# hormes/koordinator

Measured on AMD Instinct MI355X. Metric: pod×node Filter+Score evals/sec + pods/sec at 50k nodes, 1/2/4/8 GPUs, higher is better.
Workload: dtype int64

## Files before the change

koordinator_amd/csrc/gs_commit_spec.hip:

```cpp
#include <hip/hip_runtime.h>
#include <stdint.h>

#include "gs_eval_dev.h"

namespace gs {

constexpr int SP_WAVES = 8, SP_THREADS = 64 * SP_WAVES;
constexpr int SP_LAG = 12;
constexpr int SP_RES0 = 2, SP_NRES = 2;
constexpr int SP_RS0 = SP_RES0 + SP_NRES, SP_TABLES = SP_WAVES - SP_RS0;
constexpr int SP_W_VERIFY = 4;
__device__ __forceinline__ int sp_reserve_index(int wv) { return wv == 2 ? 0 : wv == 3 ? 1 : -1; }
__device__ __forceinline__ int sp_rescore_index(int wv) { return wv == 1 ? 0 : wv >= 5 ? wv - 4 : -1; }
constexpr int SP_JOBQ = 24;
constexpr int SP_HASH = 128;
static_assert(SP_HASH >= MAX_BATCH && (SP_HASH & (SP_HASH - 1)) == 0,
              "the node -> slot hash must hold every dirty slot (its insertion probes until a free entry)");
constexpr int SP_FRESH = 1, SP_FITERR = 2, SP_SLOW = 4, SP_OFFSHARD = 8;
constexpr int SP_PRED_GE = 16, SP_PRED_GT = 32;
constexpr uint32_t SP_SPIN_LIMIT = 1u << 24;
constexpr int SP_NST = 62, SP_STRIDE = 64;
constexpr int16_t SO_UNKNOWN = -2;
constexpr int16_t SO_UNLISTED = -3;

// ... 146 lines not shown
  int32_t* hkey = L.hkey;
  int16_t* hval = L.hval;
  Job* jobq = L.jobq;

  const uint64_t rt0 = __builtin_amdgcn_s_memrealtime();
  if (a.prev && a.prev[1] != 1) {
    if (tid == 0) { a.committed[0] = -1; a.committed[1] = 0; a.committed[3] = 0; a.committed[4] = 0; }
    return;
  }
  if (a.xerr && a.xerr[0]) {
    if (tid == 0) { a.committed[0] = 0; a.committed[1] = 0; a.committed[2] = 0; a.committed[3] = COMMIT_ERR_XTAG; a.committed[4] = 0; }
    return;
  }
  for (int i = tid; i < B; i += SP_THREADS) {
    pods(i) = a.pods[i];
    done_ver[i] = -1;
    has_row[i] = 0;
    rescored[i] = 0;
    jobs_left[i] = 0;
    jobs_all[i] = 0;
    resv[i] = 0;
  }
  for (int i = tid; i < SP_HASH; i += SP_THREADS) { hkey[i] = -1; hval[i] = -1; }
  for (int i = tid; i < B; i += SP_THREADS) tiebreak_records(a.seed, a.seq[i], a.tb + (size_t)i * TB_N);
  if (tid == 0) {
    s_decided = 0; s_stop = 0; s_parked = 0; s_finish = 0; s_cut_at = -1; s_err = 0; s_werr = 0;
    for (int k = 0; k < SP_NRES; ++k) { s_jq_head[k] = 0; s_jq_tail[k] = 0; }
    s_verified = 0; s_rb_req = 0; s_end_at = B; s_vend = -1; s_vcut = 0;
    s_committed = 0; s_hostcut = 0; s_nd = 0;
    s_snap = 0; s_prep_done = 0; s_reprep = 0;
  }
  __syncthreads();


  auto load_hdr = [&](int p, Hdr& o) {
    const LevelHdr* h = hdr_ptr(a, 0, p);
    const LevelExt* x = reinterpret_cast<const LevelExt*>(a.xbase + (size_t)a.bmax * LCAP * 4 +
                                                          (size_t)a.bmax * sizeof(LevelHdr)) + p;
    o.nlev = x->nlev;
    o.feas = h->feasible;
    o.next = x->next;
    o.hs = lane < MAXLEV ? h->score[lane] : lane < LEVALL ? x->score[lane - MAXLEV] : -1;
    o.hc = lane < MAXLEV ? h->count[lane] : lane < LEVALL ? x->count[lane - MAXLEV] : 0;
    o.lh = list_ptr(a, 0, p)[lane];
    o.tbv = a.tb[(size_t)p * TB_N + (lane & (TB_N - 1))];
  };
  auto tb_pos = [&](int p, int32_t tbv, int64_t T) -> int64_t {
// ... 1362 lines not shown
      for (int i = lane; i < (int)(sizeof(CpuStateDev) / 8); i += 64) d2[i] = s2[i];
      WAVE_FENCE();
    }
  }
  __syncthreads();
  const int nd = s_err ? 0 : s_nd, committed = s_err ? 0 : s_committed;
  for (int e = tid; e < nd * ROW_I64; e += SP_THREADS) {
    const int s = e / ROW_I64, j = e % ROW_I64;
    if (has_row[s] && row_word_mutable(j)) m.c64(kRowCol[j])[drows[s].node] = reinterpret_cast<const int64_t*>(&drows[s])[j];
  }
  for (int s = tid; s < nd; s += SP_THREADS)
    if (has_row[s]) m.c32(C_FREE_PODS)[drows[s].node] = drows[s].free_pods;
  constexpr int NW = 8 + 11 + 11 + 1;
  if (numa_on)
    for (int e = tid; e < nd * NW; e += SP_THREADS) {
      const int sl = e / NW, j = e % NW;
      if (!has_row[sl]) continue;
      const uint32_t node = drows[sl].node;
      if (j < 8) m.c64(C_ZRAW_CPU0 + j)[node] = (&drows[sl].nr.zraw_cpu[0])[j];
      else if (j < 19) m.c32(C_NFLAGS2 + (j - 8))[node] = reinterpret_cast<const int32_t*>(&drows[sl].nr.nflags2)[j - 8];
      else if (j < 30) m.c64(C_CPU_UN0 + (j - 19))[node] = reinterpret_cast<const int64_t*>(&cst[sl])[j - 19];
      else m.c32(C_CPU_META)[node] = (int32_t)cst[sl].meta;
    }
  for (int i = tid; i < committed; i += SP_THREADS) a.out[i].feasible = (uint32_t)final_F[i];
  if (ST && lane == 0)
    for (int i = 0; i < SP_NST; ++i)
      if (st_acc[i])
        atomicAdd(reinterpret_cast<unsigned long long*>(&a.stamps[wv * SP_STRIDE + i]), (unsigned long long)st_acc[i]);
  if (tid == 0) {
    a.committed[0] = committed;
    a.committed[1] = (committed == B && !s_hostcut && !s_err) ? 1 : 0;
    a.committed[2] = s_endwhy;
    a.committed[3] = s_err;
    a.committed[4] = (int32_t)(__builtin_amdgcn_s_memrealtime() - rt0);
  }
}

template <bool STAMPS, bool SPLIT>
static void spec_launch(const CommitArgs& a, hipStream_t st) {
  hipLaunchKernelGGL((commit_spec_kernel<STAMPS, SPLIT>), dim3(1), dim3(SP_THREADS), spec_smem_bytes(a.npods), st, a);
}

hipError_t launch_commit_spec(const CommitArgs& a, hipStream_t st) {
  const bool split = a.nranks <= 1 && a.npods >= 32;
  if (a.stamps) {
    if (split) spec_launch<true, true>(a, st);
// ... 26 lines not shown
```

koordinator_amd/csrc/gs_engine.cpp:

```cpp
#include <hip/hip_runtime.h>
#include <rccl/rccl.h>

#include <algorithm>
#include <chrono>
#include <cmath>
#include <cstdarg>
#include <cstdio>
#include <cstdlib>
#include <cstring>
#include <map>
#include <string>
#include <unordered_map>
#include <unordered_set>
#include <vector>
#include <condition_variable>
#include <deque>
#include <memory>
#include <mutex>
#include <thread>
#include <atomic>

#include "../../include/gpuscore.h"
#include "gs_ext.h"
#include "gs_kernels.h"
// ... 130 lines not shown
  PlacementDev* h_out = nullptr;
  int32_t* h_committed = nullptr;
  uint32_t* h_stage_idx = nullptr;
  int64_t* h_stage_rows = nullptr;
  uint8_t* h_xchg_send = nullptr;
  uint8_t* h_xchg_recv = nullptr;
  hipEvent_t ev[8] = {};
  struct Slot {
    int16_t* d_S = nullptr;
    uint8_t* d_aff = nullptr;
    hipEvent_t ev_go = nullptr, ev_evdone = nullptr;
    PodVec* d_pods = nullptr;
    uint64_t* d_seq = nullptr;
    PlacementDev* d_out = nullptr;
    int32_t* d_committed = nullptr;
    PodVec* h_pods = nullptr;
    uint64_t* h_seq = nullptr;
    PlacementDev* h_out = nullptr;
    int32_t* h_committed = nullptr;
    hipEvent_t ev[6] = {};
    bool untimed = false;
    uint8_t* d_lst = nullptr;
    uint32_t* d_hist = nullptr;
  } slot[2];
  bool cand_overlap = false;
  uint8_t* d_lst = nullptr;
  uint32_t* d_hist = nullptr;
  uint32_t* d_cscratch = nullptr;
  int cur_slot = 0;
  std::vector<HostNode> nodes;
  std::vector<uint8_t> row_dirty;
  std::vector<uint32_t> dirty_list;
  std::unordered_map<uint64_t, uint32_t> uid_node;
  std::unordered_map<uint64_t, int> metric_names;
  int64_t now = 0;
  bool prep_stale = true;
  Profile pf{};
  int max_score = 0;
  int nranks = 1, rank = 0;
  uint32_t n0 = 0, n1 = 0;
  bool sgather = false;
  uint32_t e0 = 0, e1 = 0;
  uint32_t sx_per = 0, sx_pld = 0;
  size_t sx_bytes = 0;
  uint8_t* d_sx_send = nullptr;
  uint8_t* d_sx_recv = nullptr;
// ... 927 lines not shown
    if (c->cb) {
      HIP_TRY(c, hipHostMalloc(&c->h_sx_send, c->sx_bytes, hipHostMallocDefault));
      HIP_TRY(c, hipHostMalloc(&c->h_sx_recv, c->sx_bytes * c->nranks, hipHostMallocDefault));
    }
  }
  if (!c->d_xsmall) HIP_TRY(c, hipMalloc(&c->d_xsmall, XSMALL * (1 + MAX_RANKS)));
  if (!c->h_xsmall) HIP_TRY(c, hipHostMalloc(&c->h_xsmall, XSMALL * MAX_RANKS, hipHostMallocDefault));
  if (const char* sk = env_str("GS_DEBUG_XCHG_SKEW")) {
    long r = -1;
    unsigned long long b = 0;
    if (sscanf(sk, "%ld:%llu", &r, &b) == 2) { c->dbg_xskew_rank = r; c->dbg_xskew_batch = b; }
  }
  return GS_OK;
}


void bind_slot(gs_ctx* c, int s) {
  const gs_ctx::Slot& x = c->slot[s];
  c->d_S = x.d_S; c->d_aff = x.d_aff;
  c->d_pods = x.d_pods; c->d_seq = x.d_seq; c->d_out = x.d_out; c->d_committed = x.d_committed;
  c->h_pods = x.h_pods; c->h_seq = x.h_seq; c->h_out = x.h_out; c->h_committed = x.h_committed;
  for (int i = 0; i < 6; ++i) c->ev[i] = x.ev[i];
  c->d_lst = x.d_lst; c->d_hist = x.d_hist;
  c->cur_slot = s;
}

constexpr int GS_REDO = 1;
constexpr size_t COMMITTED_BYTES = 32;

constexpr int SHORT_BATCH = 32;
bool direct_batch(const gs_ctx* c, int b, bool speculative) {
  return !speculative && b <= SHORT_BATCH && lvl_ranks(c) == 1;
}

bool cand_overlapped(const gs_ctx* c) {
  return c->cand_overlap && lvl_ranks(c) == 1 && !c->window_k && c->d_lst;
}

CommitArgs commit_args(gs_ctx* c, int b) {
  CommitArgs a{};
  a.m = c->mv;
  a.pods = c->d_pods;
  a.seq = c->d_seq;
  a.npods = b;
  a.nranks = lvl_ranks(c);
  a.shard_size = (c->N + a.nranks - 1) / a.nranks;
  a.xbase = a.nranks == 1 ? (cand_overlapped(c) ? c->d_lst : c->d_xchg_send)
                            : commit_spec_selected(c->window_k) ? c->d_xmerged : c->d_xchg_recv;
  a.xblock = c->xchg_bytes;
  a.bmax = c->B;
  a.pf = c->pf;
  a.seed = c->cfg.seed;
  a.forced_node = -1;
  a.out = c->d_out;
  a.committed = c->d_committed;
  a.stamps = c->d_stamps;
  a.topos = c->d_topos;
  a.aff = c->d_aff;
  a.ld = c->ld;
  a.own0 = c->n0;
  a.own1 = c->n1;
  a.S = a.nranks == 1 ? c->d_S : nullptr;
  a.S_own = c->d_S;
  a.window_k = c->window_k;
  a.start = c->next_start;
  a.nnodes = c->N;
  a.tb = c->d_tb;
  a.xerr = c->sgather ? c->d_xerr + (XERR_BYTES / 4) * c->cur_slot : c->nranks > 1 ? c->d_xerr : nullptr;
  return a;
}

int launch_batch(gs_ctx* c, int b, const int32_t* prev, const PlacementDev* prev_out = nullptr, int prev_b = 0) {
  const bool ovl = cand_overlapped(c);
  uint8_t* lblk = ovl ? c->d_lst : c->d_xchg_send;
  uint32_t* d_lists = reinterpret_cast<uint32_t*>(lblk);
  LevelHdr* d_hdrs = reinterpret_cast<LevelHdr*>(lblk + lists_bytes(c->B, c->lstride));
  LevelExt* d_ext = reinterpret_cast<LevelExt*>(lblk + lists_bytes(c->B, c->lstride) + (size_t)c->B * sizeof(LevelHdr));
  int prod_cols = 0;
  for (int i = 0; i < b; ++i) prod_cols |= (c->h_pods[i].flags & PF_PROD_SCORE) ? 1 : 0;
  uint32_t len = c->n1 - c->n0;
  if (c->numa_on && (c->numa_idx_stale || c->numa_idx_lo != c->e0 || c->numa_idx_hi != c->e1)) {
    std::vector<uint32_t> idx;
    for (uint32_t n = c->e0; n < c->e1; ++n)
      if (c->numa[n].cfg.numa_topology_policy != GS_NUMA_POLICY_NONE) idx.push_back(n);
    if (c->d_numa_idx) {
      HIP_TRY(c, host_wait_stream(c->st));
      HIP_TRY(c, host_wait_stream(c->st_ev));
      (void)hipFree(c->d_numa_idx);
      c->d_numa_idx = nullptr;
    }
// ... 21 lines not shown
  hipStream_t se = direct ? c->st : c->st_ev;
  hipStream_t rb = b >= SHORT_BATCH ? c->st_rb : c->st;
  const bool untimed = direct && rb == c->st;
  c->slot[c->cur_slot].untimed = untimed;
  if (!untimed) HIP_TRY(c, hipEventRecord(c->ev[0], se));
  if (c->sgather) {
    const uint32_t pld = c->sx_pld;
    uint8_t* blk = c->d_sx_send + c->sx_bytes * c->cur_slot;
    uint8_t* rcv = c->d_sx_recv + c->sx_bytes * c->nranks * c->cur_slot;
    HIP_TRY(c, launch_eval(c->mv, c->d_pods, b, c->pf, c->e0, c->e1, reinterpret_cast<int16_t*>(blk), pld, prod_cols,
                           c->d_numa_idx, c->numa_n, blk + (size_t)b * pld * 2, se, c->st2, c->ev_fork, c->ev_join,
                           c->slab_mv.i64 ? &c->slab_mv : nullptr));
    if (!untimed) HIP_TRY(c, hipEventRecord(c->ev[1], se));
    const size_t bytes = ((size_t)b * pld * 3 + sizeof(XTag) + 255) / 256 * 256;
    if (int rc = exchange(c, XSITE_SCORES, blk, rcv, bytes, nullptr, se)) return rc;
    HIP_TRY(c, launch_unpack_scores(rcv, bytes, c->nranks, b, c->sx_per, pld, c->N, c->d_S, c->d_aff, c->ld,
                                    c->d_xerr + (XERR_BYTES / 4) * c->cur_slot, se));
  } else {
    HIP_TRY(c, launch_eval(c->mv, c->d_pods, b, c->pf, c->n0, c->n1, c->d_S, c->ld, prod_cols, c->d_numa_idx, c->numa_n,
                           c->d_aff, se, c->st2, c->ev_fork, c->ev_join, c->slab_mv.i64 ? &c->slab_mv : nullptr));
    if (!untimed) HIP_TRY(c, hipEventRecord(c->ev[1], se));
  }
  const bool fix = ovl && prev && prev_b > 0;
  if (ovl) {
    CandPatch cp{};
    cp.extra = fix ? prev_b : 0;
    cp.hist = fix ? c->d_hist : nullptr;
    HIP_TRY(c, launch_cand(c->d_S, c->ld, len, c->n0, b, c->max_score, c->lstride, d_lists, d_hdrs, d_ext, se, &cp,
                           c->d_cscratch));
  }
  if (!direct) {
    HIP_TRY(c, hipEventRecord(sl.ev_evdone, c->st_ev));
    HIP_TRY(c, hipStreamWaitEvent(c->st, sl.ev_evdone, 0));
  } else {
    HIP_TRY(c, hipEventRecord(sl.ev_evdone, c->st));
    HIP_TRY(c, hipStreamWaitEvent(c->st_ev, sl.ev_evdone, 0));
  }
  if (fix) {
    CandPatch cp{c->mv, c->d_pods, c->pf, c->n0, c->n1, prod_cols, 0, c->d_aff, prev_out, prev};
    cp.extra = prev_b;
    cp.hist = c->d_hist;
    HIP_TRY(c, launch_fix_levels(c->d_S, c->ld, b, c->max_score, c->lstride, d_lists, d_hdrs, d_ext, cp, c->st));
  }
  const bool fused = prev && prev_b > 0 && !c->window_k;
  if (!ovl && prev && !fused)
    HIP_TRY(c, launch_patch(c->mv, c->d_pods, b, c->pf, c->n0, c->n1, c->d_S, c->ld, prod_cols, c->d_aff, prev_out,
                            prev, prev_b, c->st));
  if (!c->window_k && !ovl) {
    CandPatch cp{c->mv, c->d_pods, c->pf, c->n0, c->n1, prod_cols, 1, c->d_aff, prev_out, prev};
    HIP_TRY(c, launch_cand(c->d_S, c->ld, len, c->n0, b, c->max_score, c->lstride, d_lists, d_hdrs, d_ext, c->st,
                           fused ? &cp : nullptr, c->d_cscratch));
  }
  if (lvl_ranks(c) > 1) {
    int rc = exchange(c, XSITE_LEVELS, c->d_xchg_send, c->d_xchg_recv, c->xchg_bytes);
    if (rc) return rc;
    if (!commit_spec_selected(c->window_k)) return fail(c, GS_EUNSUPPORTED, "several ranks need the speculative commit");
    HIP_TRY(c, launch_merge_levels(c->d_xchg_recv, c->xchg_bytes, c->nranks, b, c->B, c->lstride, c->d_xmerged,
                                   c->d_xerr, c->st));
  }
  CommitArgs a = commit_args(c, b);
  a.prev = prev;
  ++c->xbatch;
  HIP_TRY(c, launch_commit(a, c->st));
  if (!untimed) HIP_TRY(c, hipEventRecord(c->ev[4], c->st));
  if (rb != c->st) HIP_TRY(c, hipStreamWaitEvent(rb, c->ev[4], 0));
  HIP_TRY(c, hipMemcpyAsync(c->h_committed, c->d_committed, COMMITTED_BYTES, hipMemcpyDeviceToHost, rb));
  HIP_TRY(c, hipMemcpyAsync(c->h_out, c->d_out, sizeof(PlacementDev) * b, hipMemcpyDeviceToHost, rb));
  HIP_TRY(c, hipEventRecord(c->ev[5], rb));
  return GS_OK;
}

int finish_batch(gs_ctx* c, int b, bool clobbered, int* committed_out) {
  uint32_t len = c->n1 - c->n0;
  {
    Where w_(c, "finish_batch: the batch's readback event");
    HIP_TRY(c, host_wait_event(c->ev[5]));
  }
  flush_exchange_times(c);
  const bool untimed = c->slot[c->cur_slot].untimed;
  if (!untimed) c->stats.eval_ms += ev_ms(c->ev[0], c->ev[1]);
  {
    const double cm = (double)(uint32_t)c->h_committed[4] * 1e-5;
    c->stats.commit_ms += cm;
    if (!untimed) c->stats.cand_ms += std::max(0.0, ev_ms(c->ev[1], c->ev[4]) - cm);
// ... 682 lines not shown
  if ((e = hipEventCreateWithFlags(&c->ev_fork, hipEventDisableTiming)) != hipSuccess) return bail("hipEventCreate", e);
  if ((e = hipEventCreateWithFlags(&c->ev_join, hipEventDisableTiming)) != hipSuccess) return bail("hipEventCreate", e);
  for (int i = 0; i < 6; ++i)
    if ((e = hipEventCreate(&c->ev[i])) != hipSuccess) return bail("hipEventCreate", e);
  size_t np = c->npad;
  if ((e = hipMalloc(&c->d_i64, np * NUM_I64_COLS * 8)) != hipSuccess) return bail("hipMalloc mirror", e);
  if ((e = hipMalloc(&c->d_i32, np * NUM_I32_COLS * 4)) != hipSuccess) return bail("hipMalloc mirror", e);
  (void)hipMemset(c->d_i64, 0, np * NUM_I64_COLS * 8);
  (void)hipMemset(c->d_i32, 0, np * NUM_I32_COLS * 4);
  c->mv.i64 = c->d_i64;
  c->mv.i32 = c->d_i32;
  c->mv.npad = (uint32_t)np;
  c->ld = c->npad;
  static_assert(sizeof(PodVec) % 8 == 0 && sizeof(PlacementDev) % 8 == 0, "staging layout");
  if ((e = hipMalloc(&c->d_pods, (sizeof(PodVec) + 8) * c->B)) != hipSuccess) return bail("hipMalloc", e);
  c->d_seq = reinterpret_cast<uint64_t*>(c->d_pods + c->B);
  if ((e = hipMalloc(&c->d_S, (size_t)c->B * c->ld * 2)) != hipSuccess) return bail("hipMalloc S", e);
  if ((e = hipMalloc(&c->d_aff, (size_t)c->B * c->ld)) != hipSuccess) return bail("hipMalloc aff", e);
  size_t xb = xchg_block_bytes(c->B, LCAP);
  if ((e = hipMalloc(&c->d_xchg_send, xb)) != hipSuccess) return bail("hipMalloc", e);
  c->xchg_bytes = xb;
  if ((e = hipMalloc(&c->d_committed, COMMITTED_BYTES + sizeof(PlacementDev) * c->B)) != hipSuccess) return bail("hipMalloc", e);
  c->d_out = reinterpret_cast<PlacementDev*>(c->d_committed + COMMITTED_BYTES / 4);
  if ((e = hipMalloc(&c->d_tb, sizeof(int32_t) * TB_N * c->B)) != hipSuccess) return bail("hipMalloc", e);
  if ((e = hipMalloc(&c->d_rowstat, sizeof(RowStat) * (1 + MAX_RANKS))) != hipSuccess) return bail("hipMalloc", e);
  if ((e = hipMalloc(&c->d_sel, 4 * (1 + MAX_RANKS))) != hipSuccess) return bail("hipMalloc", e);
  c->stage_cap = std::min<uint32_t>(c->N, 65536);
  if ((e = hipMalloc(&c->d_stage_rows, (size_t)(8 * ROW_WORDS + 4) * c->stage_cap)) != hipSuccess) return bail("hipMalloc", e);
  if ((e = hipHostMalloc(&c->h_stage_rows, (size_t)(8 * ROW_WORDS + 4) * c->stage_cap, hipHostMallocDefault)) != hipSuccess)
    return bail("hipHostMalloc", e);
  if ((e = hipHostMalloc(&c->h_pods, (sizeof(PodVec) + 8) * c->B, hipHostMallocDefault)) != hipSuccess)
    return bail("hipHostMalloc", e);
  c->h_seq = reinterpret_cast<uint64_t*>(c->h_pods + c->B);
  if ((e = hipHostMalloc(&c->h_committed, COMMITTED_BYTES + sizeof(PlacementDev) * c->B, hipHostMallocDefault)) != hipSuccess)
    return bail("hipHostMalloc", e);
  c->h_out = reinterpret_cast<PlacementDev*>(c->h_committed + COMMITTED_BYTES / 4);
  if ((e = hipHostMalloc(&c->h_xchg_send, xb, hipHostMallocDefault)) != hipSuccess) return bail("hipHostMalloc", e);
  (void)hipMemset(c->d_S, 0xff, (size_t)c->B * c->ld * 2);
  {
    for (auto& sl : c->slot) {
      if ((e = hipEventCreateWithFlags(&sl.ev_go, hipEventDisableTiming)) != hipSuccess) return bail("hipEventCreate", e);
      if ((e = hipEventCreateWithFlags(&sl.ev_evdone, hipEventDisableTiming)) != hipSuccess) return bail("hipEventCreate", e);
    }
    gs_ctx::Slot& s0 = c->slot[0];
    s0.d_S = c->d_S; s0.d_aff = c->d_aff;
    s0.d_pods = c->d_pods; s0.d_seq = c->d_seq; s0.d_out = c->d_out; s0.d_committed = c->d_committed;
    s0.h_pods = c->h_pods; s0.h_seq = c->h_seq; s0.h_out = c->h_out; s0.h_committed = c->h_committed;
    for (int i = 0; i < 6; ++i) s0.ev[i] = c->ev[i];
    gs_ctx::Slot& s1 = c->slot[1];
    if ((e = hipMalloc(&s1.d_S, (size_t)c->B * c->ld * 2)) != hipSuccess) return bail("hipMalloc S", e);
    if ((e = hipMalloc(&s1.d_aff, (size_t)c->B * c->ld)) != hipSuccess) return bail("hipMalloc aff", e);
    (void)hipMemset(s1.d_S, 0xff, (size_t)c->B * c->ld * 2);
    if ((e = hipMalloc(&s1.d_pods, (sizeof(PodVec) + 8) * c->B)) != hipSuccess) return bail("hipMalloc", e);
    s1.d_seq = reinterpret_cast<uint64_t*>(s1.d_pods + c->B);
    if ((e = hipMalloc(&s1.d_committed, COMMITTED_BYTES + sizeof(PlacementDev) * c->B)) != hipSuccess) return bail("hipMalloc", e);
    s1.d_out = reinterpret_cast<PlacementDev*>(s1.d_committed + COMMITTED_BYTES / 4);
    if ((e = hipHostMalloc(&s1.h_pods, (sizeof(PodVec) + 8) * c->B, hipHostMallocDefault)) != hipSuccess)
      return bail("hipHostMalloc", e);
    s1.h_seq = reinterpret_cast<uint64_t*>(s1.h_pods + c->B);
    if ((e = hipHostMalloc(&s1.h_committed, COMMITTED_BYTES + sizeof(PlacementDev) * c->B, hipHostMallocDefault)) != hipSuccess)
      return bail("hipHostMalloc", e);
    s1.h_out = reinterpret_cast<PlacementDev*>(s1.h_committed + COMMITTED_BYTES / 4);
    for (int i = 0; i < 6; ++i)
      if ((e = hipEventCreate(&s1.ev[i])) != hipSuccess) return bail("hipEventCreate", e);
    c->cand_overlap = !env_off("GS_CAND_OVERLAP");
    if (c->cand_overlap)
      for (auto& sl : c->slot) {
        if ((e = hipMalloc(&sl.d_lst, xb)) != hipSuccess) return bail("hipMalloc", e);
        if ((e = hipMalloc(&sl.d_hist, (size_t)4 * c->B * (MAX_SCORE_LIMIT + 1))) != hipSuccess) return bail("hipMalloc", e);
      }
    c->d_lst = s0.d_lst;
    c->d_hist = s0.d_hist;
  }
  if ((e = hipMalloc(&c->d_cscratch, cand_split_scratch_bytes())) != hipSuccess) return bail("hipMalloc", e);
  c->host_timing = env_on("GS_HOST_TIMING");
  if (env_on("GS_COMMIT_STAMPS")) {
    if ((e = hipMalloc(&c->d_stamps, 8 * 524)) != hipSuccess) return bail("hipMalloc", e);
    (void)hipMemset(c->d_stamps, 0, 8 * 524);
    set_cand_stamps(c->d_stamps + 512);
  }
  if ((e = hipDeviceSynchronize()) != hipSuccess) return bail("hipDeviceSynchronize", e);
  c->stats.node_row_bytes = 3 * 8 + 4 + 2 * 8 + 2 * 8 + 2 * 8 + 2 * 8 + 4 + (c->numa_on ? 18 * 8 + 12 * 4 : 0);
  if (const double lim = env_num("GS_WATCHDOG_S", 0.0); lim > 0) c->watchdog = std::thread(watchdog_loop, c, lim);
  *out = c;
  return GS_OK;
}

int gs_destroy(gs_ctx* c) {
  if (!c) return GS_EINVAL;
  async_stop(c);
  if (c->watchdog.joinable()) {
    c->wd_stop.store(true);
// ... 124 lines not shown
      fprintf(stderr, " | s26 (full-row resolution, per such pod) %.0f", st[18] ? (double)st[26] / (double)st[18] : 0.0);
      fprintf(stderr, " | policy-row rescoring: %llu pods, %.0f ticks per pair (thread 128)\n",
              (unsigned long long)st[12], st[12] ? (double)st[13] / st[12] : 0.0);
    }
    (void)hipFree(c->d_stamps);
  }
  if (c->comm) ncclCommDestroy(c->comm);
  if (c->lg_ready) (void)hipEventDestroy(c->lg_ready);
  if (c->lg_done) (void)hipEventDestroy(c->lg_done);
  for (hipEvent_t ev : c->x_ev) (void)hipEventDestroy(ev);
  if (c->st) (void)host_wait_stream(c->st);
  if (c->st_ev) (void)host_wait_stream(c->st_ev);
  if (c->st_rb) (void)host_wait_stream(c->st_rb);
  if (c->slot[0].d_pods) bind_slot(c, 0);
  {
    gs_ctx::Slot& s1 = c->slot[1];
    for (auto& sl : c->slot) {
      if (sl.ev_go) (void)hipEventDestroy(sl.ev_go);
      if (sl.ev_evdone) (void)hipEventDestroy(sl.ev_evdone);
    }
      for (auto& sl : c->slot) {
      if (sl.d_lst) (void)hipFree(sl.d_lst);
      if (sl.d_hist) (void)hipFree(sl.d_hist);
      sl.d_lst = nullptr;
      sl.d_hist = nullptr;
    }
    c->d_lst = nullptr;
    c->d_hist = nullptr;
    if (c->d_cscratch) (void)hipFree(c->d_cscratch);
    c->d_cscratch = nullptr;
    void* d1[] = {s1.d_pods, s1.d_committed, s1.d_S, s1.d_aff};
    for (void* p : d1)
      if (p) (void)hipFree(p);
    void* h1[] = {s1.h_pods, s1.h_committed};
    for (void* p : h1)
      if (p) (void)hipHostFree(p);
    for (auto& ev : s1.ev)
      if (ev) (void)hipEventDestroy(ev);
  }
  void* dev[] = {c->d_xerr, c->d_xsmall,
                 c->d_i64, c->d_i32, c->d_pods, c->d_S, c->d_xchg_send, c->d_xchg_recv, c->d_xmerged,
                 c->d_committed, c->d_rowstat, c->d_sel, c->d_stage_idx, c->d_stage_rows, c->d_numa_idx, c->d_xnuma_idx,
                 c->d_topos, c->d_aff, c->d_tb, c->d_sx_send, c->d_sx_recv};
  for (void* p : dev)
    if (p) (void)hipFree(p);
  void* host[] = {c->h_sx_send, c->h_sx_recv, c->h_xsmall, c->h_pods, c->h_committed, c->h_stage_idx, c->h_stage_rows, c->h_xchg_send,
                  c->h_xchg_recv};
  for (void* p : host)
// ... 1075 lines not shown
```

koordinator_amd/csrc/gs_kernels.h:

```cpp
#pragma once
#include <hip/hip_runtime.h>
#include <stddef.h>
#include <stdint.h>

#include "gs_cpuset_dev.h"
#include "gs_layout.h"

namespace gs {

constexpr int MAX_BATCH = 128;
constexpr int MAX_RANKS = 8;
constexpr int MAXLEV = 8;
constexpr int LCAP = 2048;
constexpr int XCAP = 256;
constexpr int PODS_PER_BLOCK = 16;
constexpr int MAX_SCORE_LIMIT = 2047;
constexpr int ROW_WORDS = NUM_I64_COLS + NUM_I32_COLS;
constexpr uint8_t AFF_RECOMPUTE = 0xFF;

struct MirrorView {
  int64_t* i64;
  int32_t* i32;
  uint32_t npad;
#ifdef __HIPCC__
// ... 52 lines not shown
  const uint8_t* xbase;
  size_t xblock;
  int bmax;
  Profile pf;
  uint64_t seed;
  int32_t forced_node;
  int32_t forced_score;
  int64_t forced_ties;
  int32_t forced_feasible;
  PlacementDev* out;
  int32_t* committed;
  uint64_t* stamps;
  const TopoDev* topos;
  const uint8_t* aff;
  uint32_t ld;
  uint32_t own0, own1;
  const int16_t* S;
  const int16_t* S_own;
  const int32_t* prev;
  uint32_t window_k;
  uint32_t start;
  uint32_t nnodes;
  int32_t* tb;
  const int32_t* xerr;
};
constexpr int TB_N = 32;

hipError_t set_kernel_attributes();
hipError_t launch_node_prep(const MirrorView& m, uint32_t n0, uint32_t n1, int64_t now, int32_t filter_expired,
                            int32_t has_exp, int64_t exp_ns, hipStream_t st);
hipError_t launch_node_prep_idx(const MirrorView& m, const uint32_t* idx, uint32_t n, int64_t now, int32_t filter_expired,
                                int32_t has_exp, int64_t exp_ns, hipStream_t st);
hipError_t launch_eval(const MirrorView& m, const PodVec* pods, int npods, const Profile& pf, uint32_t n0, uint32_t n1,
                       int16_t* S, uint32_t ld, int prod_cols, const uint32_t* numa_idx, uint32_t numa_n,
                       uint8_t* aff, hipStream_t st, hipStream_t st2 = nullptr, hipEvent_t fork = nullptr,
                       hipEvent_t join = nullptr,
                       const MirrorView* slab = nullptr);
hipError_t launch_patch(const MirrorView& m, const PodVec* pods, int npods, const Profile& pf, uint32_t n0, uint32_t n1,
                        int16_t* S, uint32_t ld, int prod_cols, uint8_t* aff, const PlacementDev* prev_out,
                        const int32_t* prev_committed, int prev_npods, hipStream_t st);
hipError_t launch_eval_full(const MirrorView& m, const PodVec* pods, int npods, const Profile& pf, uint32_t N,
                            int16_t* scores, uint16_t* codes, int16_t* plugin, int prod_cols, hipStream_t st);
void set_cand_stamps(uint64_t* p);
struct CandPatch {
  MirrorView m;
  const PodVec* pods;
  Profile pf;
  uint32_t n0, n1;
  int prod_cols, on;
  uint8_t* aff;
  const PlacementDev* prev_out;
  const int32_t* prev_committed;
  int extra;
  uint32_t* hist;
};
constexpr int CS_GMAX = 64, CS_MAXB = 32;
size_t cand_split_scratch_bytes();
hipError_t launch_cand(int16_t* S, uint32_t ld, uint32_t len, uint32_t n0, int npods, int max_score, int lcap,
                       uint32_t* lists, LevelHdr* hdrs, LevelExt* ext, hipStream_t st, const CandPatch* patch = nullptr,
                       uint32_t* split_scratch = nullptr);
hipError_t launch_fix_levels(int16_t* S, uint32_t ld, int npods, int max_score, int lcap, uint32_t* lists,
                             LevelHdr* hdrs, LevelExt* ext, const CandPatch& cp, hipStream_t st);
struct XTag {
  uint32_t magic;
  uint32_t site;
  uint64_t seq;
  uint64_t batch;
  int32_t rank;
  uint32_t bytes;
};
static_assert(sizeof(XTag) == 32, "XTag layout");
constexpr uint32_t XTAG_MAGIC = 0x31585347u;
enum : uint32_t { XSITE_LEVELS = 1, XSITE_ROWSTAT = 2, XSITE_SELECT = 3, XSITE_SCORES = 4, XSITE_RUNS = 5 };
constexpr int32_t COMMIT_ERR_XTAG = 90;
constexpr int XERR_TAGS = 8;
constexpr size_t XERR_BYTES = 4 * XERR_TAGS + sizeof(XTag) * MAX_RANKS;
hipError_t launch_write_tag(uint8_t* dst, const XTag& t, hipStream_t st);
hipError_t launch_merge_levels(const uint8_t* xin, size_t xblock, int nranks, int npods, int bmax, int lstride,
                               uint8_t* xout, int32_t* xerr, hipStream_t st);
hipError_t launch_unpack_scores(const uint8_t* xin, size_t xblock, int nranks, int npods, uint32_t per, uint32_t pld,
                                uint32_t N, int16_t* S, uint8_t* aff, uint32_t ld, int32_t* xerr, hipStream_t st);
size_t commit_smem_bytes(int B);
bool commit_spec_selected(uint32_t window_k);
// ... 21 lines not shown
```

koordinator_amd/csrc/gs_kernels.hip:

```cpp
#include <hip/hip_runtime.h>
#include <stdint.h>

#include <cstdio>
#include <vector>

#include "gs_eval_dev.h"

namespace gs {

__device__ __forceinline__ uint32_t node_prep_flags(uint32_t sf, int64_t update_time, int64_t now, int32_t filter_expired,
                                                    int32_t has_exp, int64_t exp_ns) {
  bool exists = sf & SF_METRIC;
  bool expired = !exists || !(sf & SF_UPDATE_TIME) || (exp_ns > 0 && now - update_time >= exp_ns);
  bool skip_filter = !exists || (filter_expired && has_exp && expired);
  uint32_t df = 0;
  if (!skip_filter) {
    const uint32_t npd = ((sf & SF_NP_MEM) ? 1u : 0u) | ((sf & SF_NP_AGG) ? 2u : 0u);
    if (sf & SF_FAIL_NP) df |= DF_LA_FAIL_NP | npd << DF_NP_DETAIL_SHIFT;
    if (sf & SF_PROD_THR) {
      if (sf & SF_FAIL_P) df |= DF_LA_FAIL_P | (((sf & SF_P_MEM) ? 1u : 0u) << DF_P_DETAIL_SHIFT);
    } else if (sf & SF_FAIL_NP) {
      df |= DF_LA_FAIL_P | npd << DF_P_DETAIL_SHIFT;
    }
  }
// ... 258 lines not shown
      const uint32_t cb = cum + (uint32_t)(wave_incl_scan((int)c) - (int)c);
      const int nb = nlev + __popcll(nzm & lt);
      const bool stop = nz && (nb == LEVALL || cb + c > (uint32_t)lcap || cb >= target);
      const uint64_t sm = __ballot(stop);
      const int ls = sm ? __builtin_ctzll(sm) : 64;
      if (nz && lane < ls) {
        s_score[nb] = b;
        s_count[nb] = (int32_t)c;
        slot_of[b] = (int8_t)nb;
      }
      if (sm) {
        next = __builtin_amdgcn_readlane(b, ls);
        nlev += __popcll(nzm & ((1ull << ls) - 1ull));
        break;
      }
      nlev += __popcll(nzm);
      cum += (uint32_t)wave_sum((int)c);
    }
    for (int j = nlev + lane; j < LEVALL; j += 64) { s_score[j] = -1; s_count[j] = 0; }
    if (lane == 0) {
      s_nlev = nlev;
      s_next = next;
    }
  }
  __syncthreads();
  CT(2);
  const int nlev = s_nlev;
  for (int e = t; e < W * LEVALL; e += CAND_THREADS) {
    const int w = e / LEVALL, j = e % LEVALL;
    uint32_t off = 0;
    if (j < nlev) {
      for (int jj = 0; jj < j; ++jj) off += s_count[jj];
      for (int ww = 0; ww < w; ++ww) off += whist[ww * nbins + s_score[j]];
    }
    s_woff[w][j] = off;
  }
  __syncthreads();
  CT(3);
  uint32_t* out = lists + (size_t)k * lcap;
  if (nlev > 0) {
    uint32_t run_l = lane < LEVALL ? s_woff[wave][lane] : 0;
    const int thr = s_score[nlev - 1];
    auto next_step = [&](uint32_t b) {
      for (; b < we; b += 512) {
        const uint32_t st = (b - wb) / 512;
        if (st >= (uint32_t)STEPCAP || s_stepmax[wave][st] >= thr) break;
// ... 248 lines not shown
                                                                 CandPatch cp, uint64_t* stamps) {
  uint64_t ct_last = stamps ? __builtin_amdgcn_s_memtime() : 0;
  auto CT = [&](int i) {
    if (!stamps) return;
    const uint64_t t_ = __builtin_amdgcn_s_memtime();
    if (threadIdx.x == 0) atomicAdd(reinterpret_cast<unsigned long long*>(&stamps[i]), (unsigned long long)(t_ - ct_last));
    ct_last = t_;
  };
  extern __shared__ __align__(16) uint32_t smem[];
  const int nbins = max_score + 1;
  uint32_t* hist = smem;
  uint32_t* olist = smem + nbins;
  __shared__ uint32_t p_raw[MAX_BATCH], p_node[MAX_BATCH];
  __shared__ int32_t p_old[MAX_BATCH], p_new[MAX_BATCH];
  __shared__ unsigned long long m_old[LEVALL][2], m_new[LEVALL][2];
  __shared__ int32_t n_ol[LEVALL];
  __shared__ int32_t o_score[LEVALL], o_count[LEVALL], o_off[LEVALL];
  __shared__ int32_t n_score[LEVALL], n_count[LEVALL], n_off[LEVALL];
  __shared__ int32_t s_onlev, s_onext, s_ofeas, s_np, s_fd, s_nlev, s_next, s_top;
  __shared__ int32_t r_old[MAX_BATCH], r_new[MAX_BATCH], p_sidx[MAX_BATCH];
  __shared__ int32_t s_wd[2];
  int8_t* lev_of = reinterpret_cast<int8_t*>(olist + lcap);
  const int k = blockIdx.x, t = threadIdx.x, lane = t & 63;
  const int32_t node_t = t < cp.extra ? cp.prev_out[t].node : -1;
  const int npr = min(cp.prev_committed[0], MAX_BATCH);
  if (npr <= 0) return;
  __shared__ unsigned int s_ev_max[2];
  if (stamps && t < 2) s_ev_max[t] = 0;
  if (stamps) __syncthreads();
  static_assert(FIX_THREADS == 256 && MAX_BATCH <= 128, "fix_levels_kernel: waves 0-1 evaluate, 2-3 load");
  if (t >= FIX_THREADS - 64) {
    const LevelHdr& h = hdrs[k];
    const LevelExt& x = ext[k];
    const int onl = x.nlev;
    const int j = lane;
    int sc = -1, cnt = 0;
    if (j < LEVALL) {
      sc = j < MAXLEV ? h.score[j] : x.score[j - MAXLEV];
      cnt = j < onl ? (j < MAXLEV ? h.count[j] : x.count[j - MAXLEV]) : 0;
    }
    const int incl = wave_incl_scan(cnt);
    if (j < LEVALL) {
      o_score[j] = sc;
      o_count[j] = cnt;
      o_off[j] = incl - cnt;
    }
    if (lane == 0) {
      s_onlev = onl;
      s_onext = x.next;
// ... 3 lines not shown
    }
    const int otot = onl > 0 ? __shfl(incl, onl - 1) : 0;
    const uint32_t* src = lists + (size_t)k * lcap;
    for (int e0 = 0; e0 < otot; e0 += 8 * 64) {
      uint32_t v[8];
#pragma unroll
      for (int u = 0; u < 8; ++u) {
        const int e = e0 + u * 64 + lane;
        v[u] = e < otot ? src[e] : 0u;
      }
#pragma unroll
      for (int u = 0; u < 8; ++u) {
        const int e = e0 + u * 64 + lane;
        if (e < otot) olist[e] = v[u];
      }
    }
  } else if (t >= FIX_THREADS - 128) {
    for (int b = lane; b < nbins; b += 64) hist[b] = cp.hist[(size_t)k * nbins + b];
  }
  const bool numa = (cp.pf.enabled & 0x30u) != 0;
  size_t at = 0;
  int so = -1, sn = -1, aff_v = -1;
  bool valid = false;
  if (t < npr) {
    const int32_t node = node_t;
    valid = node >= 0 && (uint32_t)node >= cp.n0 && (uint32_t)node < cp.n1;
    p_raw[t] = valid ? (uint32_t)node : 0xffffffffu;
    if (valid) {
      const uint64_t e0 = stamps ? __builtin_amdgcn_s_memtime() : 0;
      if (stamps && t == 0)
        atomicAdd(reinterpret_cast<unsigned long long*>(&stamps[10]), (unsigned long long)(e0 - ct_last));
      at = (size_t)k * ld + ((uint32_t)node - cp.n0);
      so = S[at];
      Row r;
      load_row(cp.m, (uint32_t)node, cp.prod_cols, numa, r);
      if (stamps) {
        __builtin_amdgcn_s_waitcnt(0);
        atomicMax(&s_ev_max[0], (unsigned int)(__builtin_amdgcn_s_memtime() - e0));
      }
      const PairOut o = eval_pair<false, false, true>(r, cp.pods[k], cp.pf, cp.m);
      sn = total_score(o, cp.pf);
      if (numa && ((r.nr.nflags >> NF_POLICY_SHIFT) & 3u)) aff_v = o.code ? 0 : (int)o.aff;
      if (stamps) atomicMax(&s_ev_max[1], (unsigned int)(__builtin_amdgcn_s_memtime() - e0));
    }
    r_old[t] = so;
    r_new[t] = sn;
  }
  __syncthreads();
  if (stamps && t == 0) {
    atomicAdd(reinterpret_cast<unsigned long long*>(&stamps[8]), (unsigned long long)s_ev_max[0]);
    atomicAdd(reinterpret_cast<unsigned long long*>(&stamps[9]), (unsigned long long)s_ev_max[1]);
    atomicAdd(reinterpret_cast<unsigned long long*>(&stamps[11]),
              (unsigned long long)(__builtin_amdgcn_s_memtime() - ct_last));
  }
  if (t < 128) {
    const uint32_t x = t < npr ? p_raw[t] : 0u;
    const uint32_t k0 = lane < npr ? p_raw[lane] : 0u, k1 = 64 + lane < npr ? p_raw[64 + lane] : 0u;
    int rank = 0;
#pragma unroll
    for (int i = 0; i < 64; ++i) {
      const uint32_t y0 = __builtin_amdgcn_readlane(k0, i), y1 = __builtin_amdgcn_readlane(k1, i);
      rank += (i < npr && (y0 < x || (y0 == x && i < t))) ? 1 : 0;
      rank += (64 + i < npr && (y1 < x || (y1 == x && 64 + i < t))) ? 1 : 0;
    }
    if (t < npr) p_sidx[rank] = t;
  }
  __syncthreads();
  bool keep = false;
  int idx = 0, wpre = 0;
  uint32_t xs = 0;
  if (t < 2 * 64) {
    if (t < npr) {
      idx = p_sidx[t];
      xs = p_raw[idx];
      keep = xs != 0xffffffffu && (t == 0 || p_raw[p_sidx[t - 1]] != xs);
    }
    const uint64_t m = __ballot(keep);
    wpre = __popcll(m & ((1ull << lane) - 1ull));
    if (lane == 0) s_wd[t >> 6] = __popcll(m);
  }
  __syncthreads();
  if (keep) {
    const int pos = (t >= 64 ? s_wd[0] : 0) + wpre;
    const int o_ = r_old[idx], n_ = r_new[idx];
    p_node[pos] = xs;
    p_old[pos] = o_;
    p_new[pos] = n_;
    if (o_ >= 0) atomicSub(&hist[o_], 1u);
    if (n_ >= 0) atomicAdd(&hist[n_], 1u);
    const int fd = (n_ >= 0 ? 1 : 0) - (o_ >= 0 ? 1 : 0);
    if (fd) atomicAdd(&s_fd, fd);
    atomicMax(&s_top, n_);
  }
  if (t == 0) s_np = s_wd[0] + s_wd[1];
  __syncthreads();
  CT(5);
  const int np = s_np;
  if (t < 64) {
    const uint32_t target = (uint32_t)k + 1;
// ... 1117 lines not shown
  hipLaunchKernelGGL(patch_kernel, dim3(prev_npods), dim3(128), 0, st, m, pods, npods, pf, n0, n1, S, ld, prod_cols, aff,
                     prev_out, prev_committed);
  return hipGetLastError();
}

hipError_t launch_eval_full(const MirrorView& m, const PodVec* pods, int npods, const Profile& pf, uint32_t N,
                            int16_t* scores, uint16_t* codes, int16_t* plugin, int prod_cols, hipStream_t st) {
  uint32_t grid = (N + 255) / 256;
  hipLaunchKernelGGL(eval_full_kernel, dim3(grid), dim3(256), 0, st, m, pods, npods, pf, N, scores, codes, plugin,
                     prod_cols);
  return hipGetLastError();
}

static size_t cand_smem_bytes(int max_score) {
  size_t nb = (size_t)max_score + 1;
  return nb * 4 * CAND_WAVES + nb * 4 + ((nb + 15) & ~(size_t)15);
}

static uint64_t* g_cand_stamps = nullptr;
void set_cand_stamps(uint64_t* p) { g_cand_stamps = p; }

hipError_t launch_fix_levels(int16_t* S, uint32_t ld, int npods, int max_score, int lcap, uint32_t* lists,
                             LevelHdr* hdrs, LevelExt* ext, const CandPatch& cp, hipStream_t st) {
  if (lcap < 1 || lcap > LCAP || !cp.hist || max_score < 0 || max_score > MAX_SCORE_LIMIT || npods > MAX_BATCH)
    return hipErrorInvalidValue;
  const size_t smem = ((size_t)max_score + 1 + (size_t)lcap) * 4 + (size_t)max_score + 1;
  hipLaunchKernelGGL(fix_levels_kernel, dim3(npods), dim3(FIX_THREADS), smem, st, S, ld, max_score, lcap, lists, hdrs, ext,
                     cp, g_cand_stamps);
  return hipGetLastError();
}


size_t cand_split_scratch_bytes() {
  return (size_t)4 * CS_MAXB * CS_GMAX * (MAX_SCORE_LIMIT + 1 + LEVALL);
}

hipError_t launch_cand(int16_t* S, uint32_t ld, uint32_t len, uint32_t n0, int npods, int max_score, int lcap,
                       uint32_t* lists, LevelHdr* hdrs, LevelExt* ext, hipStream_t st, const CandPatch* patch,
                       uint32_t* split_scratch) {
  if (lcap < 1 || lcap > LCAP) return hipErrorInvalidValue;
  CandPatch cp{};
  if (patch) cp = *patch;
  const uint32_t lenv = (len + 511) & ~511u;
  if (split_scratch && !cp.on && !cp.hist && cp.extra == 0 && !g_cand_stamps && npods >= 1 &&
      npods <= CS_MAXB && max_score >= 0 && max_score <= MAX_SCORE_LIMIT && lenv >= 2 * 2048) {
    const uint32_t g0 = min((uint32_t)CS_GMAX, (lenv + 2047) / 2048);
    const uint32_t slice = ((lenv + g0 - 1) / g0 + 2047) & ~2047u;
    const int G = (int)((lenv + slice - 1) / slice);
    const int nbins = max_score + 1;
    uint32_t* ghist = split_scratch;
    uint32_t* offs = split_scratch + (size_t)CS_MAXB * CS_GMAX * (MAX_SCORE_LIMIT + 1);
    hipLaunchKernelGGL(cs_hist_kernel, dim3(G, npods), dim3(256), (size_t)4 * nbins, st, S, ld, lenv, nbins, slice, G,
                       ghist);
    hipLaunchKernelGGL(cs_pick_kernel, dim3(npods), dim3(256), (size_t)4 * nbins, st, ghist, nbins, G, lcap, offs, hdrs,
                       ext);
    hipLaunchKernelGGL(cs_list_kernel, dim3(G, npods), dim3(64), ((size_t)nbins + 15) & ~(size_t)15, st, S, ld, lenv,
                       n0, nbins, slice, G, lcap, offs, hdrs, ext, lists);
    return hipGetLastError();
  }
  hipLaunchKernelGGL(cand_kernel, dim3(npods), dim3(64 * CAND_WAVES), cand_smem_bytes(max_score), st, S, ld, len, n0,
                     max_score, lcap, lists, hdrs, ext, g_cand_stamps, cp);
  return hipGetLastError();
}

size_t commit_smem_bytes(int B) {
  size_t b = (size_t)B * POD_STRIDE + (size_t)B * sizeof(Row) + (size_t)B * B * 2 * 2;
  b = (b + 15) & ~(size_t)15;
  b += (size_t)HASH * 8 + 16;
  b += (size_t)B * sizeof(CpuStateDev);
  return b;
}

bool commit_spec_selected(uint32_t window_k) { return !window_k; }

hipError_t launch_commit(const CommitArgs& a, hipStream_t st) {
  if (commit_spec_selected(a.window_k)) return launch_commit_spec(a, st);
  if (a.stamps)
    hipLaunchKernelGGL(commit_kernel<true>, dim3(1), dim3(COMMIT_THREADS), commit_smem_bytes(a.npods), st, a);
  else
    hipLaunchKernelGGL(commit_kernel<false>, dim3(1), dim3(COMMIT_THREADS), commit_smem_bytes(a.npods), st, a);
  return hipGetLastError();
}

hipError_t launch_row_stats(const int16_t* S, uint32_t len, RowStat* out, hipStream_t st) {
// ... 34 lines not shown
```

Baseline: 9.261 billion.

## Precompute tiebreaks in cand kernel and hand landed rows to fix-levels

The tiebreak record generation moves out of the single-block commit kernel into an idle wave of the overlapped candidate kernel, with per-slot tiebreak buffers, so the serial commit does less work. The commit kernel also writes a compact 'landed' slab holding the committed dirty rows, ordered with NUMA-policy rows first. The next batch's fix_levels kernel reads those rows directly instead of reloading them from the column store, and its sorting logic is simplified. The commit kernel gains an extra compaction and copy phase, and fix_levels now depends on the landed slab being valid.

```diff
diff --git a/koordinator_amd/csrc/gs_commit_spec.hip b/koordinator_amd/csrc/gs_commit_spec.hip
--- a/koordinator_amd/csrc/gs_commit_spec.hip
+++ b/koordinator_amd/csrc/gs_commit_spec.hip
@@ -192,7 +192,8 @@
     resv[i] = 0;
   }
   for (int i = tid; i < SP_HASH; i += SP_THREADS) { hkey[i] = -1; hval[i] = -1; }
-  for (int i = tid; i < B; i += SP_THREADS) tiebreak_records(a.seed, a.seq[i], a.tb + (size_t)i * TB_N);
+  if (!a.tb_ready)
+    for (int i = tid; i < B; i += SP_THREADS) tiebreak_records(a.seed, a.seq[i], a.tb + (size_t)i * TB_N);
   if (tid == 0) {
     s_decided = 0; s_stop = 0; s_parked = 0; s_finish = 0; s_cut_at = -1; s_err = 0; s_werr = 0;
     for (int k = 0; k < SP_NRES; ++k) { s_jq_head[k] = 0; s_jq_tail[k] = 0; }
@@ -1601,6 +1602,45 @@
       else if (j < 30) m.c64(C_CPU_UN0 + (j - 19))[node] = reinterpret_cast<const int64_t*>(&cst[sl])[j - 19];
       else m.c32(C_CPU_META)[node] = (int32_t)cst[sl].meta;
     }
+  if (a.landed) {
+    int32_t* lpos = jobs_left;
+    int32_t* lh = reinterpret_cast<int32_t*>(a.landed);
+    for (int s = tid; s < SB; s += SP_THREADS) lpos[s] = -1;
+    __syncthreads();
+    for (int q = tid; q < committed; q += SP_THREADS)
+      if (!(dec[q].flags & SP_FITERR) && (uint32_t)dec[q].slot < (uint32_t)SB) lpos[dec[q].slot] = 0;
+    __syncthreads();
+    if (wv == 0) {
+      static_assert(SB == 128, "two slots per lane");
+      bool pol[2], non[2];
+      for (int h = 0; h < 2; ++h) {
+        const int s = h * 64 + lane;
+        const bool on = s < nd && has_row[s] && lpos[s] == 0;
+        pol[h] = on && numa_on && ((drows[s].nr.nflags >> NF_POLICY_SHIFT) & 3u);
+        non[h] = on && !pol[h];
+      }
+      const uint64_t p0 = __ballot(pol[0]), p1 = __ballot(pol[1]), n0 = __ballot(non[0]), n1 = __ballot(non[1]);
+      const int npol = __popcll(p0) + __popcll(p1);
+      WAVE_FENCE();
+      lpos[lane] = pol[0] ? __popcll(p0 & lt_mask) : non[0] ? npol + __popcll(n0 & lt_mask) : -1;
+      lpos[64 + lane] = pol[1] ? __popcll(p0) + __popcll(p1 & lt_mask)
+                               : non[1] ? npol + __popcll(n0) + __popcll(n1 & lt_mask) : -1;
+      if (lane == 0) {
+        lh[0] = npol + __popcll(n0) + __popcll(n1);
+        lh[1] = npol;
+      }
+    }
+    __syncthreads();
+    for (int s = tid; s < nd; s += SP_THREADS)
+      if (lpos[s] >= 0) lh[LANDED_NODES / 4 + lpos[s]] = (int32_t)drows[s].node;
+    constexpr int RW = (int)(sizeof(Row) / 8);
+    const uint64_t* src = reinterpret_cast<const uint64_t*>(drows);
+    uint64_t* dst = reinterpret_cast<uint64_t*>(a.landed + LANDED_ROWS);
+    for (int e = tid; e < nd * RW; e += SP_THREADS) {
+      const int s = e / RW;
+      if (lpos[s] >= 0) dst[lpos[s] * RW + (e - s * RW)] = src[e];
+    }
+  }
   for (int i = tid; i < committed; i += SP_THREADS) a.out[i].feasible = (uint32_t)final_F[i];
   if (ST && lane == 0)
     for (int i = 0; i < SP_NST; ++i)
diff --git a/koordinator_amd/csrc/gs_engine.cpp b/koordinator_amd/csrc/gs_engine.cpp
--- a/koordinator_amd/csrc/gs_engine.cpp
+++ b/koordinator_amd/csrc/gs_engine.cpp
@@ -176,6 +176,8 @@
     bool untimed = false;
     uint8_t* d_lst = nullptr;
     uint32_t* d_hist = nullptr;
+    int32_t* d_tb = nullptr;
+    uint8_t* d_landed = nullptr;
   } slot[2];
   bool cand_overlap = false;
   uint8_t* d_lst = nullptr;
@@ -1149,6 +1151,7 @@
   c->h_pods = x.h_pods; c->h_seq = x.h_seq; c->h_out = x.h_out; c->h_committed = x.h_committed;
   for (int i = 0; i < 6; ++i) c->ev[i] = x.ev[i];
   c->d_lst = x.d_lst; c->d_hist = x.d_hist;
+  c->d_tb = x.d_tb;
   c->cur_slot = s;
 }
 
@@ -1193,6 +1196,7 @@
   a.start = c->next_start;
   a.nnodes = c->N;
   a.tb = c->d_tb;
+  a.landed = c->slot[c->cur_slot].d_landed;
   a.xerr = c->sgather ? c->d_xerr + (XERR_BYTES / 4) * c->cur_slot : c->nranks > 1 ? c->d_xerr : nullptr;
   return a;
 }
@@ -1260,12 +1264,16 @@
     if (!untimed) HIP_TRY(c, hipEventRecord(c->ev[1], se));
   }
   const bool fix = ovl && prev && prev_b > 0;
+  int32_t tb_ready = 0;
   if (ovl) {
     CandPatch cp{};
     cp.extra = fix ? prev_b : 0;
     cp.hist = fix ? c->d_hist : nullptr;
+    cp.tb = c->d_tb;
+    cp.seq = c->d_seq;
+    cp.seed = c->cfg.seed;
     HIP_TRY(c, launch_cand(c->d_S, c->ld, len, c->n0, b, c->max_score, c->lstride, d_lists, d_hdrs, d_ext, se, &cp,
-                           c->d_cscratch));
+                           c->d_cscratch, &tb_ready));
   }
   if (!direct) {
     HIP_TRY(c, hipEventRecord(sl.ev_evdone, c->st_ev));
@@ -1278,6 +1286,7 @@
     CandPatch cp{c->mv, c->d_pods, c->pf, c->n0, c->n1, prod_cols, 0, c->d_aff, prev_out, prev};
     cp.extra = prev_b;
     cp.hist = c->d_hist;
+    cp.landed = c->slot[1 - c->cur_slot].d_landed;
     HIP_TRY(c, launch_fix_levels(c->d_S, c->ld, b, c->max_score, c->lstride, d_lists, d_hdrs, d_ext, cp, c->st));
   }
   const bool fused = prev && prev_b > 0 && !c->window_k;
@@ -1298,6 +1307,7 @@
   }
   CommitArgs a = commit_args(c, b);
   a.prev = prev;
+  a.tb_ready = tb_ready;
   ++c->xbatch;
   HIP_TRY(c, launch_commit(a, c->st));
   if (!untimed) HIP_TRY(c, hipEventRecord(c->ev[4], c->st));
@@ -2026,7 +2036,7 @@
   c->xchg_bytes = xb;
   if ((e = hipMalloc(&c->d_committed, COMMITTED_BYTES + sizeof(PlacementDev) * c->B)) != hipSuccess) return bail("hipMalloc", e);
   c->d_out = reinterpret_cast<PlacementDev*>(c->d_committed + COMMITTED_BYTES / 4);
-  if ((e = hipMalloc(&c->d_tb, sizeof(int32_t) * TB_N * c->B)) != hipSuccess) return bail("hipMalloc", e);
+  if ((e = hipMalloc(&c->d_tb, sizeof(int32_t) * TB_N * c->B * 2)) != hipSuccess) return bail("hipMalloc", e);
   if ((e = hipMalloc(&c->d_rowstat, sizeof(RowStat) * (1 + MAX_RANKS))) != hipSuccess) return bail("hipMalloc", e);
   if ((e = hipMalloc(&c->d_sel, 4 * (1 + MAX_RANKS))) != hipSuccess) return bail("hipMalloc", e);
   c->stage_cap = std::min<uint32_t>(c->N, 65536);
@@ -2052,6 +2062,8 @@
     s0.h_pods = c->h_pods; s0.h_seq = c->h_seq; s0.h_out = c->h_out; s0.h_committed = c->h_committed;
     for (int i = 0; i < 6; ++i) s0.ev[i] = c->ev[i];
     gs_ctx::Slot& s1 = c->slot[1];
+    s0.d_tb = c->d_tb;
+    s1.d_tb = c->d_tb + (size_t)TB_N * c->B;
     if ((e = hipMalloc(&s1.d_S, (size_t)c->B * c->ld * 2)) != hipSuccess) return bail("hipMalloc S", e);
     if ((e = hipMalloc(&s1.d_aff, (size_t)c->B * c->ld)) != hipSuccess) return bail("hipMalloc aff", e);
     (void)hipMemset(s1.d_S, 0xff, (size_t)c->B * c->ld * 2);
@@ -2072,6 +2084,8 @@
       for (auto& sl : c->slot) {
         if ((e = hipMalloc(&sl.d_lst, xb)) != hipSuccess) return bail("hipMalloc", e);
         if ((e = hipMalloc(&sl.d_hist, (size_t)4 * c->B * (MAX_SCORE_LIMIT + 1))) != hipSuccess) return bail("hipMalloc", e);
+        if ((e = hipMalloc(&sl.d_landed, landed_slab_bytes())) != hipSuccess) return bail("hipMalloc", e);
+        (void)hipMemset(sl.d_landed, 0, landed_slab_bytes());
       }
     c->d_lst = s0.d_lst;
     c->d_hist = s0.d_hist;
@@ -2242,8 +2256,10 @@
       for (auto& sl : c->slot) {
       if (sl.d_lst) (void)hipFree(sl.d_lst);
       if (sl.d_hist) (void)hipFree(sl.d_hist);
+      if (sl.d_landed) (void)hipFree(sl.d_landed);
       sl.d_lst = nullptr;
       sl.d_hist = nullptr;
+      sl.d_landed = nullptr;
     }
     c->d_lst = nullptr;
     c->d_hist = nullptr;
diff --git a/koordinator_amd/csrc/gs_kernels.h b/koordinator_amd/csrc/gs_kernels.h
--- a/koordinator_amd/csrc/gs_kernels.h
+++ b/koordinator_amd/csrc/gs_kernels.h
@@ -98,8 +98,12 @@
   uint32_t start;
   uint32_t nnodes;
   int32_t* tb;
+  int32_t tb_ready;
+  uint8_t* landed;
   const int32_t* xerr;
 };
+constexpr size_t LANDED_NODES = 16, LANDED_ROWS = LANDED_NODES + 4 * MAX_BATCH;
+size_t landed_slab_bytes();
 constexpr int TB_N = 32;
 
 hipError_t set_kernel_attributes();
@@ -129,12 +133,16 @@
   const int32_t* prev_committed;
   int extra;
   uint32_t* hist;
+  int32_t* tb;
+  const uint64_t* seq;
+  uint64_t seed;
+  const uint8_t* landed;
 };
 constexpr int CS_GMAX = 64, CS_MAXB = 32;
 size_t cand_split_scratch_bytes();
 hipError_t launch_cand(int16_t* S, uint32_t ld, uint32_t len, uint32_t n0, int npods, int max_score, int lcap,
                        uint32_t* lists, LevelHdr* hdrs, LevelExt* ext, hipStream_t st, const CandPatch* patch = nullptr,
-                       uint32_t* split_scratch = nullptr);
+                       uint32_t* split_scratch = nullptr, int32_t* tb_written = nullptr);
 hipError_t launch_fix_levels(int16_t* S, uint32_t ld, int npods, int max_score, int lcap, uint32_t* lists,
                              LevelHdr* hdrs, LevelExt* ext, const CandPatch& cp, hipStream_t st);
 struct XTag {
diff --git a/koordinator_amd/csrc/gs_kernels.hip b/koordinator_amd/csrc/gs_kernels.hip
--- a/koordinator_amd/csrc/gs_kernels.hip
+++ b/koordinator_amd/csrc/gs_kernels.hip
@@ -304,6 +304,8 @@
       s_nlev = nlev;
       s_next = next;
     }
+  } else if (t == 64 && cp.tb) {
+    tiebreak_records(cp.seed, cp.seq[k], cp.tb + (size_t)k * TB_N);
   }
   __syncthreads();
   CT(2);
@@ -598,9 +600,12 @@
   __shared__ int32_t s_wd[2];
   int8_t* lev_of = reinterpret_cast<int8_t*>(olist + lcap);
   const int k = blockIdx.x, t = threadIdx.x, lane = t & 63;
-  const int32_t node_t = t < cp.extra ? cp.prev_out[t].node : -1;
-  const int npr = min(cp.prev_committed[0], MAX_BATCH);
-  if (npr <= 0) return;
+  if (cp.prev_committed[0] <= 0) return;
+  const int32_t* lh = reinterpret_cast<const int32_t*>(cp.landed);
+  const int nl = min(max(lh[0], 0), MAX_BATCH), npol = min(max(lh[1], 0), nl);
+  const int split = min(max(npol, nl - 64), 64);
+  const int slot_t = t < 64 ? (t < split ? t : -1) : (t < 128 && split + (t - 64) < nl ? split + (t - 64) : -1);
+  const int32_t node_t = slot_t >= 0 ? lh[LANDED_NODES / 4 + slot_t] : -1;
   __shared__ unsigned int s_ev_max[2];
   if (stamps && t < 2) s_ev_max[t] = 0;
   if (stamps) __syncthreads();
@@ -650,7 +655,7 @@
   size_t at = 0;
   int so = -1, sn = -1, aff_v = -1;
   bool valid = false;
-  if (t < npr) {
+  if (t < 128) {
     const int32_t node = node_t;
     valid = node >= 0 && (uint32_t)node >= cp.n0 && (uint32_t)node < cp.n1;
     p_raw[t] = valid ? (uint32_t)node : 0xffffffffu;
@@ -660,13 +665,12 @@
         atomicAdd(reinterpret_cast<unsigned long long*>(&stamps[10]), (unsigned long long)(e0 - ct_last));
       at = (size_t)k * ld + ((uint32_t)node - cp.n0);
       so = S[at];
-      Row r;
-      load_row(cp.m, (uint32_t)node, cp.prod_cols, numa, r);
+      const Row r = reinterpret_cast<const Row*>(cp.landed + LANDED_ROWS)[slot_t];
       if (stamps) {
         __builtin_amdgcn_s_waitcnt(0);
         atomicMax(&s_ev_max[0], (unsigned int)(__builtin_amdgcn_s_memtime() - e0));
       }
-      const PairOut o = eval_pair<false, false, true>(r, cp.pods[k], cp.pf, cp.m);
+      const PairOut o = eval_pair<false, true, true>(r, cp.pods[k], cp.pf, cp.m);
       sn = total_score(o, cp.pf);
       if (numa && ((r.nr.nflags >> NF_POLICY_SHIFT) & 3u)) aff_v = o.code ? 0 : (int)o.aff;
       if (stamps) atomicMax(&s_ev_max[1], (unsigned int)(__builtin_amdgcn_s_memtime() - e0));
@@ -682,27 +686,25 @@
               (unsigned long long)(__builtin_amdgcn_s_memtime() - ct_last));
   }
   if (t < 128) {
-    const uint32_t x = t < npr ? p_raw[t] : 0u;
-    const uint32_t k0 = lane < npr ? p_raw[lane] : 0u, k1 = 64 + lane < npr ? p_raw[64 + lane] : 0u;
+    const uint32_t x = p_raw[t];
+    const uint32_t k0 = p_raw[lane], k1 = p_raw[64 + lane];
     int rank = 0;
 #pragma unroll
     for (int i = 0; i < 64; ++i) {
       const uint32_t y0 = __builtin_amdgcn_readlane(k0, i), y1 = __builtin_amdgcn_readlane(k1, i);
-      rank += (i < npr && (y0 < x || (y0 == x && i < t))) ? 1 : 0;
-      rank += (64 + i < npr && (y1 < x || (y1 == x && 64 + i < t))) ? 1 : 0;
-    }
-    if (t < npr) p_sidx[rank] = t;
+      rank += ((y0 < x || (y0 == x && i < t))) ? 1 : 0;
+      rank += ((y1 < x || (y1 == x && 64 + i < t))) ? 1 : 0;
+    }
+    p_sidx[rank] = t;
   }
   __syncthreads();
   bool keep = false;
   int idx = 0, wpre = 0;
   uint32_t xs = 0;
   if (t < 2 * 64) {
-    if (t < npr) {
-      idx = p_sidx[t];
-      xs = p_raw[idx];
-      keep = xs != 0xffffffffu && (t == 0 || p_raw[p_sidx[t - 1]] != xs);
-    }
+    idx = p_sidx[t];
+    xs = p_raw[idx];
+    keep = xs != 0xffffffffu && (t == 0 || p_raw[p_sidx[t - 1]] != xs);
     const uint64_t m = __ballot(keep);
     wpre = __popcll(m & ((1ull << lane) - 1ull));
     if (lane == 0) s_wd[t >> 6] = __popcll(m);
@@ -1866,7 +1868,8 @@
 
 hipError_t launch_fix_levels(int16_t* S, uint32_t ld, int npods, int max_score, int lcap, uint32_t* lists,
                              LevelHdr* hdrs, LevelExt* ext, const CandPatch& cp, hipStream_t st) {
-  if (lcap < 1 || lcap > LCAP || !cp.hist || max_score < 0 || max_score > MAX_SCORE_LIMIT || npods > MAX_BATCH)
+  if (lcap < 1 || lcap > LCAP || !cp.hist || !cp.landed || max_score < 0 ||
+      max_score > MAX_SCORE_LIMIT || npods > MAX_BATCH)
     return hipErrorInvalidValue;
   const size_t smem = ((size_t)max_score + 1 + (size_t)lcap) * 4 + (size_t)max_score + 1;
   hipLaunchKernelGGL(fix_levels_kernel, dim3(npods), dim3(FIX_THREADS), smem, st, S, ld, max_score, lcap, lists, hdrs, ext,
@@ -1875,16 +1878,19 @@
 }
 
 
+size_t landed_slab_bytes() { return LANDED_ROWS + (size_t)MAX_BATCH * sizeof(Row); }
+
 size_t cand_split_scratch_bytes() {
   return (size_t)4 * CS_MAXB * CS_GMAX * (MAX_SCORE_LIMIT + 1 + LEVALL);
 }
 
 hipError_t launch_cand(int16_t* S, uint32_t ld, uint32_t len, uint32_t n0, int npods, int max_score, int lcap,
                        uint32_t* lists, LevelHdr* hdrs, LevelExt* ext, hipStream_t st, const CandPatch* patch,
-                       uint32_t* split_scratch) {
+                       uint32_t* split_scratch, int32_t* tb_written) {
   if (lcap < 1 || lcap > LCAP) return hipErrorInvalidValue;
   CandPatch cp{};
   if (patch) cp = *patch;
+  if (tb_written) *tb_written = 0;
   const uint32_t lenv = (len + 511) & ~511u;
   if (split_scratch && !cp.on && !cp.hist && cp.extra == 0 && !g_cand_stamps && npods >= 1 &&
       npods <= CS_MAXB && max_score >= 0 && max_score <= MAX_SCORE_LIMIT && lenv >= 2 * 2048) {
@@ -1904,6 +1910,7 @@
   }
   hipLaunchKernelGGL(cand_kernel, dim3(npods), dim3(64 * CAND_WAVES), cand_smem_bytes(max_score), st, S, ld, len, n0,
                      max_score, lcap, lists, hdrs, ext, g_cand_stamps, cp);
+  if (tb_written && cp.tb) *tb_written = 1;
   return hipGetLastError();
 }
 
```

Result: faster. 9.426 billion, median of 6 (+1.8%).
